# GreptimeTeam/greptimedb

Measured on AMD Instinct MI355X. Metric: TSBS DevOps ingest rows/sec (whole node), higher is better.
Workload: dtype f64; 1 GPU; model=tsbs-devops-cpu-only, global_batch=3000, seq_len=0, parallelism=region-shard dp1, scale_per_worker=100, workers=6, pool_rows=2394000, rows_shipped_cross_rank=0, wal=group-commit, no fsync, flush_mb=64, ssts_written=4, device=cuda:0

## Files before the change

### csrc/hip_ops.cpp

```cpp

#include <torch/extension.h>
#include <ATen/hip/HIPContext.h>

#include <algorithm>
#include <cmath>
#include <cstdint>
#include <tuple>
#include <vector>

#include "scatter_packed.h"

namespace gdb_hip {
void launch_ts_bucket_agg(
    const int64_t*, const int32_t*, const double*, int64_t, const int32_t*, int,
    const int32_t*, int, int64_t, int64_t, int64_t, int64_t, int, int, int64_t,
    double*, unsigned long long*, unsigned long long*, unsigned long long*,
    unsigned long long*, hipStream_t);
void launch_decode_minmax(
    const unsigned long long*, const unsigned long long*, const unsigned long long*,
    double*, double*, int64_t, hipStream_t);
void launch_filter_series_time(
    const int64_t*, const int32_t*, const int32_t*, int, int64_t, int64_t,
    int64_t, bool*, hipStream_t);
void launch_dedup_mark_last(const int32_t*, const int64_t*, int64_t, bool*, hipStream_t);
// ... 252 lines not shown
    CHECK_GPU(dst_ts[r]); CHECK_GPU(dst_se[r]); CHECK_GPU(dst_fields[r]);
    CHECK_CONTIG(dst_ts[r]); CHECK_CONTIG(dst_se[r]); CHECK_CONTIG(dst_fields[r]);
    TORCH_CHECK(dst_fields[r].dim() == 2 && dst_fields[r].size(0) >= nf,
                "region ", r, " has fewer field rows than the batch");
    TORCH_CHECK(bases[r] >= 0);
    regs.ts[r] = dst_ts[r].data_ptr<int64_t>();
    regs.se[r] = dst_se[r].data_ptr<int32_t>();
    regs.f[r] = dst_fields[r].data_ptr<double>();
    regs.stride[r] = dst_fields[r].size(1);
    regs.base[r] = bases[r];
    room[r] = std::min(std::min(dst_ts[r].numel(), dst_se[r].numel()),
                       dst_fields[r].size(1));
  }
  const uint8_t* hp = stage_pinned.data_ptr<uint8_t>();
  const int64_t* h_dst = reinterpret_cast<const int64_t*>(hp + off_dst);
  const int32_t* h_region = reinterpret_cast<const int32_t*>(hp + off_region);
  for (int64_t i = 0; i < n; i++) {
    const int32_t r = h_region[i];
    TORCH_CHECK(r >= 0 && r < R, "row ", i, ": region ", r, " out of range");
    TORCH_CHECK(h_dst[i] >= 0 && bases[r] + h_dst[i] < room[r],
                "row ", i, ": destination row beyond region ", r, " capacity");
  }
  auto stream = at::cuda::getCurrentHIPStream().stream();
  const hipError_t err = hipMemcpyAsync(
      stage_dev.data_ptr<uint8_t>(), hp, (size_t)used, hipMemcpyHostToDevice, stream);
  TORCH_CHECK(err == hipSuccess, "stage upload failed: ", hipGetErrorString(err));
  gdb_hip::launch_scatter_append_packed(
      stage_dev.data_ptr<uint8_t>(), n, (int)nf, regs, stream);
  const hipError_t lerr = hipGetLastError();
  TORCH_CHECK(lerr == hipSuccess, "scatter_append_packed launch failed: ",
              hipGetErrorString(lerr));
}

torch::Tensor rle_expand_indices(torch::Tensor runs, torch::Tensor blob,
                                 int64_t bw, int64_t n) {
  CHECK_GPU(runs); CHECK_CONTIG(runs); CHECK_GPU(blob); CHECK_CONTIG(blob);
  auto out = torch::empty({n}, blob.options().dtype(torch::kInt32));
  auto stream = at::cuda::getCurrentHIPStream().stream();
  gdb_hip::launch_rle_expand_indices(
      runs.data_ptr<int64_t>(), runs.size(0), blob.data_ptr<uint8_t>(),
      (int)bw, out.data_ptr<int32_t>(), n, stream);
  return out;
}

std::vector<torch::Tensor> gorilla_decode(torch::Tensor blob,
                                          torch::Tensor block_off,
                                          torch::Tensor out_off, int64_t n) {
  CHECK_GPU(blob); CHECK_CONTIG(blob);
  CHECK_GPU(block_off); CHECK_GPU(out_off);
  auto ts = torch::empty({n}, blob.options().dtype(torch::kInt64));
  auto vals = torch::empty({n}, blob.options().dtype(torch::kFloat64));
  auto stream = at::cuda::getCurrentHIPStream().stream();
// ... 181 lines not shown
```

### csrc/native.cpp

```cpp

#include <pybind11/pybind11.h>
#include <pybind11/numpy.h>
#include <pybind11/stl.h>

#include <cerrno>
#include <cmath>
#include <cstdint>
#include <cstring>
#include <fcntl.h>
#include <stdexcept>
#include <string>
#include <unistd.h>
#include <unordered_map>
#include <vector>

#include "ingest_core.h"

namespace py = pybind11;

static uint32_t crc_table[8][256];
static bool crc_init_done = [] {
  for (uint32_t i = 0; i < 256; i++) {
    uint32_t c = i;
    for (int k = 0; k < 8; k++) c = (c & 1) ? 0xEDB88320u ^ (c >> 1) : c >> 1;
    crc_table[0][i] = c;
  }
  for (int t = 1; t < 8; t++)
    for (uint32_t i = 0; i < 256; i++)
      crc_table[t][i] = crc_table[0][crc_table[t - 1][i] & 0xFF] ^
                        (crc_table[t - 1][i] >> 8);
  return true;
}();

static uint32_t crc32_update(uint32_t crc, const uint8_t* buf, size_t len) {
  crc = ~crc;
  while (len >= 8) {
    uint32_t lo, hi;
    std::memcpy(&lo, buf, 4);
    std::memcpy(&hi, buf + 4, 4);
    lo ^= crc;
    crc = crc_table[7][lo & 0xFF] ^ crc_table[6][(lo >> 8) & 0xFF] ^
          crc_table[5][(lo >> 16) & 0xFF] ^ crc_table[4][lo >> 24] ^
          crc_table[3][hi & 0xFF] ^ crc_table[2][(hi >> 8) & 0xFF] ^
          crc_table[1][(hi >> 16) & 0xFF] ^ crc_table[0][hi >> 24];
    buf += 8;
    len -= 8;
  }
  for (size_t i = 0; i < len; i++)
    crc = crc_table[0][(crc ^ buf[i]) & 0xFF] ^ (crc >> 8);
  return ~crc;
}

static inline uint64_t fnv1a(const char* p, size_t n) {
  uint64_t h = 1469598103934665603ULL;
  for (size_t i = 0; i < n; i++) { h ^= (uint8_t)p[i]; h *= 1099511628211ULL; }
  return h;
}


static py::capsule owner_of(void* p) {
  return py::capsule(p, [](void* q) { std::free(q); });
}

class LineParser {
 public:
  py::tuple parse(py::bytes data) {
    char* buf;
    Py_ssize_t len;
    if (PyBytes_AsStringAndSize(data.ptr(), &buf, &len) != 0)
      throw std::runtime_error("expected bytes");
    gdb_ingest::ParseSink sink;
    const size_t F0 = core_.num_fields();
    size_t nrows = 0, est = 0;
    int32_t* series = nullptr;
// ... 120 lines not shown
        py::array_t<double> a((py::ssize_t)n);
        if (n) {
          if (c < sink.col.size()) {
            std::memcpy(a.mutable_data(), sink.col[c], 8 * n);
          } else {
            std::fill(a.mutable_data(), a.mutable_data() + n, std::nan(""));
          }
        }
        fields[py::str(names[c])] = std::move(a);
      }
    }
    py::list newts;
    for (auto& [id, s] : sink.new_tagsets)
      newts.append(py::make_tuple(id, py::bytes(s)));
    return py::make_tuple(std::move(series), std::move(ts), std::move(fields),
                          std::move(newts));
  }

  gdb_ingest::LineCore core_;
};



class WalWriter {
 public:
  WalWriter() = default;
  ~WalWriter() { close_segment(); }

  void open_segment(const std::string& path) {
    close_segment();
    fd_ = ::open(path.c_str(), O_CREAT | O_WRONLY | O_APPEND, 0644);
    if (fd_ < 0) throw std::runtime_error("wal open failed: " + path + ": " + strerror(errno));
    path_ = path;
    seg_bytes_ = ::lseek(fd_, 0, SEEK_END);
  }

  void close_segment() {
    if (fd_ >= 0) { ::close(fd_); fd_ = -1; }
  }

  void append(uint64_t region_id, uint64_t seq, py::object payload) {
    char* pbuf; Py_ssize_t plen;
    Py_buffer view;
    bool have_view = false;
    if (PyBytes_Check(payload.ptr())) {
      if (PyBytes_AsStringAndSize(payload.ptr(), &pbuf, &plen) != 0)
        throw std::runtime_error("payload must be bytes");
    } else {
      if (PyObject_GetBuffer(payload.ptr(), &view, PyBUF_SIMPLE) != 0)
        throw py::error_already_set();
      have_view = true;
      pbuf = static_cast<char*>(view.buf);
      plen = view.len;
    }
    struct Release {
      Py_buffer* v;
      ~Release() { if (v) PyBuffer_Release(v); }
    } release{have_view ? &view : nullptr};
    py::gil_scoped_release rel;
    uint32_t body_len = 16 + static_cast<uint32_t>(plen);
    size_t off = buf_.size();
    buf_.resize(off + 8 + body_len);
    uint8_t* w = buf_.data() + off;
    std::memcpy(w, &body_len, 4);
    uint8_t hdr[16];
    std::memcpy(hdr, &region_id, 8);
    std::memcpy(hdr + 8, &seq, 8);
    uint32_t crc = crc32_update(0, hdr, 16);
    crc = crc32_update(crc, reinterpret_cast<uint8_t*>(pbuf), plen);
    std::memcpy(w + 4, &crc, 4);
    std::memcpy(w + 8, hdr, 16);
    std::memcpy(w + 24, pbuf, plen);
  }

  uint64_t commit(bool sync) {
    if (fd_ < 0) throw std::runtime_error("wal: no open segment");
    size_t n = buf_.size();
    if (n) {
      py::gil_scoped_release rel;
      const uint8_t* p = buf_.data();
      size_t left = n;
      while (left) {
        ssize_t w = ::write(fd_, p, left);
        if (w < 0) {
          if (errno == EINTR) continue;
          throw std::runtime_error(std::string("wal write failed: ") + strerror(errno));
        }
        p += w; left -= w;
      }
      if (sync && ::fdatasync(fd_) != 0)
        throw std::runtime_error(std::string("wal fdatasync failed: ") + strerror(errno));
    }
    buf_.clear();
    seg_bytes_ += n;
    return seg_bytes_;
  }

  uint64_t segment_bytes() const { return seg_bytes_; }

 private:
  int fd_ = -1;
  std::string path_;
  uint64_t seg_bytes_ = 0;
  std::vector<uint8_t> buf_;
};

static py::list wal_read_segment(const std::string& path) {
  py::list out;
  int fd = ::open(path.c_str(), O_RDONLY);
  if (fd < 0) throw std::runtime_error("wal open failed: " + path);
  off_t sz = ::lseek(fd, 0, SEEK_END);
  ::lseek(fd, 0, SEEK_SET);
  std::vector<uint8_t> data(sz);
  size_t got = 0;
  while (got < static_cast<size_t>(sz)) {
    ssize_t r = ::read(fd, data.data() + got, sz - got);
    if (r <= 0) break;
    got += r;
  }
  ::close(fd);
  size_t off = 0;
  while (off + 8 <= got) {
    uint32_t body_len, crc;
    std::memcpy(&body_len, data.data() + off, 4);
    std::memcpy(&crc, data.data() + off + 4, 4);
    if (body_len < 16 || off + 8 + body_len > got) break;
    const uint8_t* body = data.data() + off + 8;
    if (crc32_update(0, body, body_len) != crc) break;
    uint64_t region, seq;
    std::memcpy(&region, body, 8);
    std::memcpy(&seq, body + 8, 8);
    out.append(py::make_tuple(region, seq,
        py::bytes(reinterpret_cast<const char*>(body + 16), body_len - 16)));
    off += 8 + body_len;
  }
  return out;
}


static bool snappy_uncompress(const uint8_t* in, size_t n, std::vector<uint8_t>& out) {
  size_t ip = 0;
  uint64_t ulen = 0;
  int shift = 0;
  while (ip < n) {
    uint8_t b = in[ip++];
    ulen |= (uint64_t)(b & 0x7F) << shift;
    if (!(b & 0x80)) break;
    shift += 7;
    if (shift > 35) return false;
  }
  out.clear();
  out.reserve(ulen);
  while (ip < n) {
    const uint8_t tag = in[ip++];
    const int type = tag & 3;
    if (type == 0) {
      size_t len = (tag >> 2) + 1;
      if (len > 60) {
        const int extra = (int)len - 60;
// ... 945 lines not shown
                        std::move(counts), std::move(mins), std::move(maxs));
}

void register_pagedec(py::module_& m);

PYBIND11_MODULE(_native, m) {
  register_pagedec(m);
  m.doc() = "greptimedb_amd host-native ingest path (line parser + WAL)";
  py::class_<LineParser>(m, "LineParser")
      .def(py::init<>())
      .def("parse", &LineParser::parse)
      .def("ingest_batch", &LineParser::ingest_batch, py::arg("data"),
           py::arg("sid_region"), py::arg("sid_local"), py::arg("fmap"),
           py::arg("n_parser_fields"), py::arg("n_regions"),
           py::arg("hdr_suffix"), py::arg("durable"), py::arg("ts_scale"),
           py::arg("stage"))
      .def("num_fields", &LineParser::num_fields)
      .def("intern_capacity", &LineParser::intern_capacity)
      .def("num_series", &LineParser::num_series)
      .def("tagset_str", &LineParser::tagset_str)
      .def("field_names", &LineParser::field_names)
      .def("register_tagset", &LineParser::register_tagset)
      .def("register_field", &LineParser::register_field);
  py::class_<WalWriter>(m, "WalWriter")
      .def(py::init<>())
      .def("open_segment", &WalWriter::open_segment)
      .def("close_segment", &WalWriter::close_segment)
      .def("append", &WalWriter::append)
      .def("commit", &WalWriter::commit, py::arg("sync") = true)
      .def("segment_bytes", &WalWriter::segment_bytes);
  m.def("wal_read_segment", &wal_read_segment);
  m.def("snappy_uncompress", &py_snappy_uncompress);
  m.def("pack_str_col", &pack_str_col);
  m.def("route_ingest", &route_ingest, "K16 host-side ingest router");
  py::class_<PromWriteParser>(m, "PromWriteParser")
      .def(py::init<>())
      .def("parse", &PromWriteParser::parse, py::arg("data"), py::arg("is_snappy") = true)
      .def("num_series", &PromWriteParser::num_series);
  py::class_<OtlpMetricsParser>(m, "OtlpMetricsParser")
      .def(py::init<>())
      .def("parse", &OtlpMetricsParser::parse);
  py::class_<OtlpLogsParser>(m, "OtlpLogsParser")
      .def(py::init<>())
      .def("parse", &OtlpLogsParser::parse);
  py::class_<OtlpTraceParser>(m, "OtlpTraceParser")
      .def(py::init<>())
      .def("parse", &OtlpTraceParser::parse)
      .def("num_series", &OtlpTraceParser::num_series);
  py::class_<Tokenizer>(m, "Tokenizer")
      .def(py::init<>())
      .def("tokenize", &Tokenizer::tokenize)
      .def("term_id", &Tokenizer::term_id)
      .def("intern", &Tokenizer::intern)
// ... 5 lines not shown
```

### greptimedb_amd/engine/engine.py

```python

from __future__ import annotations

import json
import os
import queue
import threading
from dataclasses import dataclass, field

import numpy as np

from greptimedb_amd.engine.region import Region
from greptimedb_amd.engine.wal import Wal, decode_batch, encode_batch
from greptimedb_amd.models.schema import TableSchema, region_id as make_region_id
from greptimedb_amd.utils.errors import TableAlreadyExists, TableNotFound


@dataclass
class EngineConfig:
    data_dir: str = "./greptime_data"
    device: str = "cpu"
    flush_bytes: int = 512 << 20
    wal_sync: bool = False
    wal_segment_bytes: int = 256 << 20
    wal_shards: int = 1
    default_regions: int = 4
    background_flush: bool = True
    scan_mem_bytes: int = 32 << 30
    record_events: bool = False
    gc_interval_s: float = 600.0
    gc_grace_s: float = 3600.0
    cold_compress_s: float = 0.0
    global_write_buffer_bytes: int = 16 << 30


@dataclass
class TableState:
    schema: TableSchema
    regions: list = field(default_factory=list)
    append_mode: bool = False
    rule: object = None


class MitoEngine:
    def __init__(self, config: EngineConfig):
        self.config = config
        os.makedirs(config.data_dir, exist_ok=True)
        self.tables: dict[str, TableState] = {}
        self.next_table_id = 1024
        self._ddl_lock = threading.Lock()
        self._catalog_path = os.path.join(config.data_dir, "catalog.json")
        self.wal = Wal(os.path.join(config.data_dir, "wal"),
                       segment_bytes=config.wal_segment_bytes,
                       sync_on_commit=config.wal_sync,
                       shards=config.wal_shards)
        self._flush_q: queue.Queue = queue.Queue()
        self._flusher = None
        self.write_listeners: list = []
        self.flush_listeners: list = []
        self.mirror_listeners: list = []
        from greptimedb_amd.utils.memquota import MemoryQuota
        self.scan_quota = MemoryQuota(config.scan_mem_bytes)
        self._load_catalog()
        self._replay_wal()
# ... 274 lines not shown
                mem.max_ts = mx if mem.max_ts is None else max(mem.max_ts, mx)
                region.last_seq = max(region.last_seq, seqs[k])
                region.row_seq += m
        finally:
            for r in reversed(ordered):
                r.lock.release()
        if self.mirror_listeners and n:
            fnames = table.regions[0].field_names
            for k, region in enumerate(regions):
                if int(counts[k]) == 0:
                    continue
                rows = np.flatnonzero(region_of == k)
                for cb in self.mirror_listeners:
                    cb(table, region, series_codes[rows], ts_ms[rows],
                       fields[:, rows], fnames)
        if self.write_listeners and n:
            lo, hi = int(np.min(ts_ms)), int(np.max(ts_ms))
            for cb in self.write_listeners:
                cb(table.schema.name, lo, hi, n)
        return True

    def write_regions_fused(self, table: TableState, slot, n: int, nf: int,
                            counts, mins, maxs, payloads: list,
                            durable: bool = True) -> None:
        import torch
        from greptimedb_amd.ops import cpu_ref
        from greptimedb_amd.ops import kernels as ops

        regions: list[Region] = table.regions
        counts = [int(c) for c in counts]
        seqs = [0] * len(regions)
        if durable:
            for k, p in enumerate(payloads):
                if p is not None:
                    seqs[k] = self.wal.append(regions[k].region_id, p)
        ordered = sorted(regions, key=lambda r: r.region_id)
        for r in ordered:
            r.lock.acquire()
        try:
            bases = []
            for k, region in enumerate(regions):
                mem = region.memtable
                if mem.nf < nf:
                    mem.add_fields(nf - mem.nf)
                need = mem.len + counts[k]
                if need > mem.cap:
                    mem._grow(need)
                bases.append(mem.len)
            dst_ts = [r.memtable.ts for r in regions]
            dst_se = [r.memtable.series for r in regions]
            dst_f = [r.memtable.fields for r in regions]
            if slot.dev is not None:
                ops.scatter_append_packed(slot.host, slot.dev, n, nf, bases,
                                          dst_ts, dst_se, dst_f)
                if slot.event is not None:
                    slot.event.record()
            else:
                ts_h, f_h, do_h, se_h, ro_h = cpu_ref.packed_segments(
                    slot.host, n, nf)
                dev = self.config.device
                dst = do_h + torch.tensor(bases, dtype=torch.int64)[ro_h.long()]
                ops.scatter_append(ts_h.to(dev), se_h.to(dev), f_h.to(dev),
                                   ro_h.to(dev), dst.to(dev),
                                   dst_ts, dst_se, dst_f)
            for k, region in enumerate(regions):
                m = counts[k]
                if m == 0:
                    continue
                mem = region.memtable
                mem.len = bases[k] + m
                mn, mx = int(mins[k]), int(maxs[k])
                mem.min_ts = mn if mem.min_ts is None else min(mem.min_ts, mn)
                mem.max_ts = mx if mem.max_ts is None else max(mem.max_ts, mx)
                region.last_seq = max(region.last_seq, seqs[k])
                region.row_seq += m
        finally:
            for r in reversed(ordered):
                r.lock.release()
        if (self.mirror_listeners or self.write_listeners) and n:
            ts_h, f_h, _do, se_h, ro_h = (
                t.numpy() for t in cpu_ref.packed_segments(slot.host, n, nf))
            if self.mirror_listeners:
                fnames = table.regions[0].field_names
                for k, region in enumerate(regions):
                    if counts[k] == 0:
                        continue
                    rows = np.flatnonzero(ro_h == k)
                    for cb in self.mirror_listeners:
                        cb(table, region, se_h[rows], ts_h[rows],
                           f_h[:, rows], fnames)
            if self.write_listeners:
                lo, hi = int(np.min(ts_h)), int(np.max(ts_h))
                for cb in self.write_listeners:
                    cb(table.schema.name, lo, hi, n)
# ... 203 lines not shown
```

### greptimedb_amd/engine/ingest.py

```python

from __future__ import annotations

import weakref

import numpy as np

from greptimedb_amd import _native
from greptimedb_amd.engine.engine import MitoEngine, TableState
from greptimedb_amd.engine.series import tsid_hash
from greptimedb_amd.models.schema import ColumnSchema, DataType, SemanticType, TableSchema


def parse_tagset(key: bytes) -> tuple[str, list[tuple[str, str]]]:
    parts = key.decode().split(",")
    measurement = parts[0]
    tags = []
    for p in parts[1:]:
        if "=" in p:
            k, v = p.split("=", 1)
            tags.append((k, v))
    return measurement, tags


STAGE_RING = 3
# ... 18 lines not shown
                slot.event.synchronize()
            except Exception:
                pass
            slot.busy = False


class Ingestor:
    def __init__(self, engine: MitoEngine, default_regions: int | None = None,
                 append_mode: bool = True, durable: bool = True,
                 rank: int = 0, world: int = 1, exchange=None):
        self.engine = engine
        self.parser = _native.LineParser()
        self.append_mode = append_mode
        self.durable = durable
        self.default_regions = default_regions or engine.config.default_regions
        self.rank = rank
        self.world = world
        self.exchange = exchange
        self._remote_cache: dict[bytes, tuple[int, int]] = {}
        self._remote_lock = __import__("threading").Lock()
        self._bulk = engine.config.device.startswith("cuda")
        self._fused = True
        self._packed = True
        self._ring: list[_StageSlot] = []
        self._ring_pos = 0
        self._fused_st = None
        self._fused_lut = None
        weakref.finalize(self, _drain_ring, self._ring)
        self._cap = 1024
        self.sid_region = np.full(self._cap, -1, dtype=np.int32)
        self.sid_local = np.full(self._cap, -1, dtype=np.int32)
        self.sid_rank = np.full(self._cap, -1, dtype=np.int32)
        self.sid_key = np.empty(self._cap, dtype=object)
        self.flat_regions: list = []
        self._region_key: dict = {}
        self._table_field_map: dict = {}
        self._wal_suffix_cache: dict = {}
        self._flat_ridx_cache = None
        self._flat_ridx_table = None
        self.rows_ingested = 0
        self.rows_shipped = 0

    def _flat_region(self, st: TableState, region_idx: int) -> int:
        key = (st.schema.name, region_idx)
        idx = self._region_key.get(key)
        if idx is None:
# ... 172 lines not shown
        lut = self._fused_lut or self._build_fused_lut(st0)
        fmap = cached[0]
        nf = len(fmap)
        suffix = self._wal_suffix(st0)
        if not self._ring:
            self._grow_ring(1 << 16)
        res = None
        for _attempt in range(2):
            slot = self._next_slot()
            res = self.parser.ingest_batch(
                data, lut[0], lut[1], fmap, nparse, len(regions), suffix,
                self.durable, int(ts_scale_to_ns), slot.np)
            if res[0] != 2:
                break
            self._grow_ring(int(res[1]))
        if res[0] == 2:
            raise RuntimeError("ingest stage block still too small after growing")
        if res[0] == 1:
            return res[1]
        _, n, counts, mins, maxs, payloads = res
        if n == 0:
            return 0
        engine = self.engine
        engine.write_regions_fused(st0, slot, n, nf, counts, mins, maxs,
                                   payloads, durable=self.durable)
        slot.busy = slot.event is not None
        self._ring_pos = (self._ring_pos + 1) % len(self._ring)
        if self.durable:
            engine.commit_wal()
        engine.maybe_flush()
        self.rows_ingested += n
        return n

    def ingest_lines(self, data: bytes, ts_scale_to_ns: int = 1) -> int:
        if self._bulk and self._fused:
            got = self._ingest_fused(data, ts_scale_to_ns)
            if isinstance(got, int):
                return got
            series, ts_ns, fields, new_tagsets = got
        else:
            series, ts_ns, fields, new_tagsets = self.parser.parse(data)
        n = len(series)
        if n == 0:
            return 0
        self._check_epoch()
        for sid, key in new_tagsets:
            self._register_tagset(sid, key)
        rank_of = self.sid_rank[series]
        if bool((rank_of < 0).any()):
            for sid in np.unique(series[rank_of < 0]):
                self._register_tagset(int(sid), self.parser.tagset_str(int(sid)))
# ... 212 lines not shown
```

### greptimedb_amd/engine/wal.py

```python

from __future__ import annotations

import heapq
import json
import os
import re
import struct
import threading

import numpy as np

from greptimedb_amd import _native


def encode_batch(series: np.ndarray, ts_ms: np.ndarray, fields: np.ndarray,
                 field_names: list[str], new_series: list[tuple[int, bytes]],
                 str_cols: dict[str, list] | None = None) -> bytes:
    str_cols = str_cols or {}
    bin_cols = [name for name, vals in str_cols.items()
                if any(isinstance(v, (bytes, bytearray)) for v in vals)]
    hdr = json.dumps({
        "n": int(len(ts_ms)),
        "fields": field_names,
        "strs": list(str_cols),
# ... 93 lines not shown
    def _shard_of(self, region_id: int) -> _Shard:
        return self.shards[region_id % len(self.shards)]

    def append(self, region_id: int, payload: bytes) -> int:
        with self._lock:
            seq = self.next_seq
            self.next_seq += 1
            self.region_last[region_id] = seq
        sh = self._shard_of(region_id)
        with sh.lock:
            sh.writer.append(region_id, seq, payload)
            sh.dirty = True
        return seq

    def commit(self):
        for sh in self.shards:
            if not sh.dirty:
                continue
            with sh.lock:
                if not sh.dirty:
                    continue
                size = sh.writer.commit(self.sync_on_commit)
                sh.dirty = False
                if size >= self.segment_bytes:
                    sh.writer.close_segment()
                    sh.writer.open_segment(sh.seg_path(self.next_seq))

    def replay(self):
        def shard_stream(shard_idx):
            for seg in self.segments(shard_idx):
                for region, seq, payload in _native.wal_read_segment(
                        os.path.join(self.dir, seg)):
                    yield seq, seg, region, payload

        streams = [shard_stream(i) for i in range(len(self.shards))]
        present = {int(_SEG_RE.match(f).group(2) or 0) for f in self.segments()}
        for extra in sorted(present - set(range(len(self.shards)))):
            streams.append(shard_stream(extra))
        for seq, seg, region, payload in heapq.merge(*streams):
            yield seg, region, seq, payload

    def purge_before(self, seq: int):
        for sh in range(len(self.shards)):
            segs = self.segments(sh)
            for i, seg in enumerate(segs[:-1]):
                nxt_first = int(_SEG_RE.match(segs[i + 1]).group(1))
                if nxt_first <= seq:
                    os.unlink(os.path.join(self.dir, seg))

    def close(self):
        for sh in self.shards:
            if sh.writer is None:
                continue
            try:
                sh.writer.commit(self.sync_on_commit)
            except RuntimeError:
                pass
            sh.writer.close_segment()
            sh.writer = None
        self.shards = []
```

Measured before the change: 14.70 million rows/s.

## Batch WAL append+commit natively, add CLMUL CRC, release GIL around upload

Moves the WAL writer into a shared C++ header and adds a native append-and-commit call that frames and writes all region payloads of a fused batch in one GIL-free pass, replacing the per-region Python append loop plus a separate commit. Adds a PCLMUL-based CRC32 path for payloads of 64 bytes or more, caches the sorted region order and converts count/min/max arrays with tolist. It also releases the GIL around the H2D stage copy and scatter launch. The WAL path now writes immediately per batch instead of buffering, and rotation and sync semantics change.

Result: faster. 16.64 million rows/s (median of 6 runs) (+13.2%).

```diff
diff --git a/csrc/hip_ops.cpp b/csrc/hip_ops.cpp
--- a/csrc/hip_ops.cpp
+++ b/csrc/hip_ops.cpp
@@ -298,12 +298,17 @@
                 "row ", i, ": destination row beyond region ", r, " capacity");
   }
   auto stream = at::cuda::getCurrentHIPStream().stream();
-  const hipError_t err = hipMemcpyAsync(
-      stage_dev.data_ptr<uint8_t>(), hp, (size_t)used, hipMemcpyHostToDevice, stream);
+  uint8_t* dp = stage_dev.data_ptr<uint8_t>();
+  hipError_t err = hipSuccess, lerr = hipSuccess;
+  {
+    py::gil_scoped_release nogil;
+    err = hipMemcpyAsync(dp, hp, (size_t)used, hipMemcpyHostToDevice, stream);
+    if (err == hipSuccess) {
+      gdb_hip::launch_scatter_append_packed(dp, n, (int)nf, regs, stream);
+      lerr = hipGetLastError();
+    }
+  }
   TORCH_CHECK(err == hipSuccess, "stage upload failed: ", hipGetErrorString(err));
-  gdb_hip::launch_scatter_append_packed(
-      stage_dev.data_ptr<uint8_t>(), n, (int)nf, regs, stream);
-  const hipError_t lerr = hipGetLastError();
   TORCH_CHECK(lerr == hipSuccess, "scatter_append_packed launch failed: ",
               hipGetErrorString(lerr));
 }
diff --git a/csrc/native.cpp b/csrc/native.cpp
--- a/csrc/native.cpp
+++ b/csrc/native.cpp
@@ -15,41 +15,11 @@
 #include <vector>
 
 #include "ingest_core.h"
+#include "wal_core.h"
 
 namespace py = pybind11;
 
-static uint32_t crc_table[8][256];
-static bool crc_init_done = [] {
-  for (uint32_t i = 0; i < 256; i++) {
-    uint32_t c = i;
-    for (int k = 0; k < 8; k++) c = (c & 1) ? 0xEDB88320u ^ (c >> 1) : c >> 1;
-    crc_table[0][i] = c;
-  }
-  for (int t = 1; t < 8; t++)
-    for (uint32_t i = 0; i < 256; i++)
-      crc_table[t][i] = crc_table[0][crc_table[t - 1][i] & 0xFF] ^
-                        (crc_table[t - 1][i] >> 8);
-  return true;
-}();
-
-static uint32_t crc32_update(uint32_t crc, const uint8_t* buf, size_t len) {
-  crc = ~crc;
-  while (len >= 8) {
-    uint32_t lo, hi;
-    std::memcpy(&lo, buf, 4);
-    std::memcpy(&hi, buf + 4, 4);
-    lo ^= crc;
-    crc = crc_table[7][lo & 0xFF] ^ crc_table[6][(lo >> 8) & 0xFF] ^
-          crc_table[5][(lo >> 16) & 0xFF] ^ crc_table[4][lo >> 24] ^
-          crc_table[3][hi & 0xFF] ^ crc_table[2][(hi >> 8) & 0xFF] ^
-          crc_table[1][(hi >> 16) & 0xFF] ^ crc_table[0][hi >> 24];
-    buf += 8;
-    len -= 8;
-  }
-  for (size_t i = 0; i < len; i++)
-    crc = crc_table[0][(crc ^ buf[i]) & 0xFF] ^ (crc >> 8);
-  return ~crc;
-}
+using gdb_wal::crc32_update;
 
 static inline uint64_t fnv1a(const char* p, size_t n) {
   uint64_t h = 1469598103934665603ULL;
@@ -216,119 +186,112 @@
 
 
 
-class WalWriter {
- public:
-  WalWriter() = default;
-  ~WalWriter() { close_segment(); }
-
-  void open_segment(const std::string& path) {
-    close_segment();
-    fd_ = ::open(path.c_str(), O_CREAT | O_WRONLY | O_APPEND, 0644);
-    if (fd_ < 0) throw std::runtime_error("wal open failed: " + path + ": " + strerror(errno));
-    path_ = path;
-    seg_bytes_ = ::lseek(fd_, 0, SEEK_END);
-  }
-
-  void close_segment() {
-    if (fd_ >= 0) { ::close(fd_); fd_ = -1; }
-  }
-
-  void append(uint64_t region_id, uint64_t seq, py::object payload) {
-    char* pbuf; Py_ssize_t plen;
-    Py_buffer view;
-    bool have_view = false;
-    if (PyBytes_Check(payload.ptr())) {
-      if (PyBytes_AsStringAndSize(payload.ptr(), &pbuf, &plen) != 0)
+struct PayloadView {
+  const uint8_t* p = nullptr;
+  size_t n = 0;
+  Py_buffer view;
+  bool have_view = false;
+  py::object owner;
+
+  PayloadView() = default;
+  PayloadView(const PayloadView&) = delete;
+  PayloadView& operator=(const PayloadView&) = delete;
+  ~PayloadView() { if (have_view) PyBuffer_Release(&view); }
+
+  void acquire(PyObject* o) {
+    owner = py::reinterpret_borrow<py::object>(o);
+    if (PyBytes_Check(o)) {
+      char* b; Py_ssize_t len;
+      if (PyBytes_AsStringAndSize(o, &b, &len) != 0)
         throw std::runtime_error("payload must be bytes");
+      p = reinterpret_cast<const uint8_t*>(b);
+      n = (size_t)len;
     } else {
-      if (PyObject_GetBuffer(payload.ptr(), &view, PyBUF_SIMPLE) != 0)
+      if (PyObject_GetBuffer(o, &view, PyBUF_SIMPLE) != 0)
         throw py::error_already_set();
       have_view = true;
-      pbuf = static_cast<char*>(view.buf);
-      plen = view.len;
-    }
-    struct Release {
-      Py_buffer* v;
-      ~Release() { if (v) PyBuffer_Release(v); }
-    } release{have_view ? &view : nullptr};
+      p = static_cast<const uint8_t*>(view.buf);
+      n = (size_t)view.len;
+    }
+  }
+};
+
+static void wal_writer_append(gdb_wal::WalWriter& w, uint64_t region_id,
+                              uint64_t seq, py::object payload) {
+  PayloadView v;
+  v.acquire(payload.ptr());
+  py::gil_scoped_release rel;
+  w.append(region_id, seq, v.p, v.n);
+}
+
+static py::list wal_append_commit(py::list writers,
+                                  std::vector<uint64_t> region_ids,
+                                  std::vector<uint64_t> seqs,
+                                  py::list payloads, bool sync) {
+  const size_t m = (size_t)py::len(writers);
+  if (region_ids.size() != m || seqs.size() != m || (size_t)py::len(payloads) != m)
+    throw std::runtime_error("wal_append_commit: argument lists differ in length");
+  std::vector<gdb_wal::WalWriter*> w(m);
+  std::vector<py::object> writer_refs(m);
+  std::vector<PayloadView> views(m);
+  for (size_t i = 0; i < m; i++) {
+    writer_refs[i] = writers[i];
+    w[i] = py::cast<gdb_wal::WalWriter*>(writer_refs[i]);
+    if (w[i] == nullptr)
+      throw std::runtime_error("wal_append_commit: writer is None");
+    views[i].acquire(py::object(payloads[i]).ptr());
+  }
+  std::vector<uint64_t> sizes(m, 0);
+  std::string error;
+  {
     py::gil_scoped_release rel;
-    uint32_t body_len = 16 + static_cast<uint32_t>(plen);
-    size_t off = buf_.size();
-    buf_.resize(off + 8 + body_len);
-    uint8_t* w = buf_.data() + off;
-    std::memcpy(w, &body_len, 4);
-    uint8_t hdr[16];
-    std::memcpy(hdr, &region_id, 8);
-    std::memcpy(hdr + 8, &seq, 8);
-    uint32_t crc = crc32_update(0, hdr, 16);
-    crc = crc32_update(crc, reinterpret_cast<uint8_t*>(pbuf), plen);
-    std::memcpy(w + 4, &crc, 4);
-    std::memcpy(w + 8, hdr, 16);
-    std::memcpy(w + 24, pbuf, plen);
-  }
-
-  uint64_t commit(bool sync) {
-    if (fd_ < 0) throw std::runtime_error("wal: no open segment");
-    size_t n = buf_.size();
-    if (n) {
-      py::gil_scoped_release rel;
-      const uint8_t* p = buf_.data();
-      size_t left = n;
-      while (left) {
-        ssize_t w = ::write(fd_, p, left);
-        if (w < 0) {
-          if (errno == EINTR) continue;
-          throw std::runtime_error(std::string("wal write failed: ") + strerror(errno));
-        }
-        p += w; left -= w;
-      }
-      if (sync && ::fdatasync(fd_) != 0)
-        throw std::runtime_error(std::string("wal fdatasync failed: ") + strerror(errno));
-    }
-    buf_.clear();
-    seg_bytes_ += n;
-    return seg_bytes_;
-  }
-
-  uint64_t segment_bytes() const { return seg_bytes_; }
-
- private:
-  int fd_ = -1;
-  std::string path_;
-  uint64_t seg_bytes_ = 0;
-  std::vector<uint8_t> buf_;
-};
+    try {
+      std::vector<uint8_t> hdrs(m * gdb_wal::kFrameHeaderBytes);
+      for (size_t i = 0; i < m; i++)
+        gdb_wal::frame_header(hdrs.data() + i * gdb_wal::kFrameHeaderBytes,
+                              region_ids[i], seqs[i], views[i].p, views[i].n);
+      for (size_t i = 0; i < m; i++) {
+        bool last_of_writer = true;
+        for (size_t j = i + 1; j < m && last_of_writer; j++)
+          last_of_writer = w[j] != w[i];
+        sizes[i] = w[i]->append_commit(
+            hdrs.data() + i * gdb_wal::kFrameHeaderBytes, views[i].p,
+            views[i].n, sync && last_of_writer);
+      }
+    } catch (const std::exception& e) {
+      error = e.what();
+      if (error.empty()) error = "wal_append_commit failed";
+    }
+  }
+  if (!error.empty()) throw std::runtime_error(error);
+  py::list out;
+  for (size_t i = 0; i < m; i++) out.append(py::int_(sizes[i]));
+  return out;
+}
 
 static py::list wal_read_segment(const std::string& path) {
+  std::vector<uint8_t> data;
+  std::vector<gdb_wal::FrameView> frames;
+  {
+    py::gil_scoped_release rel;
+    data = gdb_wal::read_file(path);
+    frames = gdb_wal::read_frames(data.data(), data.size());
+  }
   py::list out;
-  int fd = ::open(path.c_str(), O_RDONLY);
-  if (fd < 0) throw std::runtime_error("wal open failed: " + path);
-  off_t sz = ::lseek(fd, 0, SEEK_END);
-  ::lseek(fd, 0, SEEK_SET);
-  std::vector<uint8_t> data(sz);
-  size_t got = 0;
-  while (got < static_cast<size_t>(sz)) {
-    ssize_t r = ::read(fd, data.data() + got, sz - got);
-    if (r <= 0) break;
-    got += r;
-  }
-  ::close(fd);
-  size_t off = 0;
-  while (off + 8 <= got) {
-    uint32_t body_len, crc;
-    std::memcpy(&body_len, data.data() + off, 4);
-    std::memcpy(&crc, data.data() + off + 4, 4);
-    if (body_len < 16 || off + 8 + body_len > got) break;
-    const uint8_t* body = data.data() + off + 8;
-    if (crc32_update(0, body, body_len) != crc) break;
-    uint64_t region, seq;
-    std::memcpy(&region, body, 8);
-    std::memcpy(&seq, body + 8, 8);
-    out.append(py::make_tuple(region, seq,
-        py::bytes(reinterpret_cast<const char*>(body + 16), body_len - 16)));
-    off += 8 + body_len;
-  }
+  for (const auto& f : frames)
+    out.append(py::make_tuple(
+        f.region, f.seq,
+        py::bytes(reinterpret_cast<const char*>(f.payload), f.plen)));
   return out;
+}
+
+static uint32_t py_crc32(py::object data, uint32_t init, const std::string& impl) {
+  PayloadView v;
+  v.acquire(data.ptr());
+  if (impl == "auto") return gdb_wal::crc32_update(init, v.p, v.n);
+  if (impl == "table") return gdb_wal::crc32_table(init, v.p, v.n);
+  if (impl == "clmul") return gdb_wal::crc32_clmul(init, v.p, v.n);
+  throw std::invalid_argument("crc32: impl must be auto, table or clmul");
 }
 
 
@@ -1320,13 +1283,32 @@
       .def("field_names", &LineParser::field_names)
       .def("register_tagset", &LineParser::register_tagset)
       .def("register_field", &LineParser::register_field);
-  py::class_<WalWriter>(m, "WalWriter")
+  py::class_<gdb_wal::WalWriter>(m, "WalWriter")
       .def(py::init<>())
-      .def("open_segment", &WalWriter::open_segment)
-      .def("close_segment", &WalWriter::close_segment)
-      .def("append", &WalWriter::append)
-      .def("commit", &WalWriter::commit, py::arg("sync") = true)
-      .def("segment_bytes", &WalWriter::segment_bytes);
+      .def("open_segment", &gdb_wal::WalWriter::open_segment,
+           py::call_guard<py::gil_scoped_release>())
+      .def("close_segment", &gdb_wal::WalWriter::close_segment,
+           py::arg("sync") = false, py::call_guard<py::gil_scoped_release>())
+      .def("rotate", &gdb_wal::WalWriter::rotate, py::arg("path"),
+           py::arg("sync") = false, py::call_guard<py::gil_scoped_release>())
+      .def("append", &wal_writer_append)
+      .def("commit", &gdb_wal::WalWriter::commit, py::arg("sync") = true,
+           py::call_guard<py::gil_scoped_release>())
+      .def("segment_bytes", &gdb_wal::WalWriter::segment_bytes,
+           py::call_guard<py::gil_scoped_release>())
+      .def("unsynced_bytes", &gdb_wal::WalWriter::unsynced_bytes,
+           py::call_guard<py::gil_scoped_release>())
+      .def("sync_count", &gdb_wal::WalWriter::sync_count,
+           py::call_guard<py::gil_scoped_release>());
+  m.def("wal_append_commit", &wal_append_commit, py::arg("writers"),
+        py::arg("region_ids"), py::arg("seqs"), py::arg("payloads"),
+        py::arg("sync") = false);
+  m.def("crc32", &py_crc32, py::arg("data"), py::arg("init") = 0,
+        py::arg("impl") = "auto");
+  m.def("crc32_have_clmul", &gdb_wal::crc32_have_clmul);
+  m.def("crc32_force_table", [](bool on) {
+    gdb_wal::crc32_force_table_flag().store(on);
+  }, "measurement switch: make the \"auto\" CRC path use the table");
   m.def("wal_read_segment", &wal_read_segment);
   m.def("snappy_uncompress", &py_snappy_uncompress);
   m.def("pack_str_col", &pack_str_col);
diff --git a/csrc/wal_core.h b/csrc/wal_core.h
--- /dev/null
+++ b/csrc/wal_core.h
@@ -0,0 +1,379 @@
+#pragma once
+
+#include <atomic>
+#include <cerrno>
+#include <cstdint>
+#include <cstring>
+#include <fcntl.h>
+#include <mutex>
+#include <stdexcept>
+#include <string>
+#include <sys/uio.h>
+#include <unistd.h>
+#include <vector>
+
+#if defined(__x86_64__) && (defined(__GNUC__) || defined(__clang__))
+#define GDB_WAL_HAVE_CLMUL_BUILD 1
+#include <immintrin.h>
+#else
+#define GDB_WAL_HAVE_CLMUL_BUILD 0
+#endif
+
+namespace gdb_wal {
+
+
+struct CrcTables {
+  uint32_t t[8][256];
+  CrcTables() {
+    for (uint32_t i = 0; i < 256; i++) {
+      uint32_t c = i;
+      for (int k = 0; k < 8; k++) c = (c & 1) ? 0xEDB88320u ^ (c >> 1) : c >> 1;
+      t[0][i] = c;
+    }
+    for (int s = 1; s < 8; s++)
+      for (uint32_t i = 0; i < 256; i++)
+        t[s][i] = t[0][t[s - 1][i] & 0xFF] ^ (t[s - 1][i] >> 8);
+  }
+};
+
+inline const CrcTables& crc_tables() {
+  static const CrcTables tables;
+  return tables;
+}
+
+inline uint32_t crc32_table_raw(uint32_t crc, const uint8_t* buf, size_t len) {
+  const auto& T = crc_tables().t;
+  while (len >= 8) {
+    uint32_t lo, hi;
+    std::memcpy(&lo, buf, 4);
+    std::memcpy(&hi, buf + 4, 4);
+    lo ^= crc;
+    crc = T[7][lo & 0xFF] ^ T[6][(lo >> 8) & 0xFF] ^
+          T[5][(lo >> 16) & 0xFF] ^ T[4][lo >> 24] ^
+          T[3][hi & 0xFF] ^ T[2][(hi >> 8) & 0xFF] ^
+          T[1][(hi >> 16) & 0xFF] ^ T[0][hi >> 24];
+    buf += 8;
+    len -= 8;
+  }
+  for (size_t i = 0; i < len; i++)
+    crc = T[0][(crc ^ buf[i]) & 0xFF] ^ (crc >> 8);
+  return crc;
+}
+
+inline uint32_t crc32_table(uint32_t crc, const uint8_t* buf, size_t len) {
+  return ~crc32_table_raw(~crc, buf, len);
+}
+
+inline bool crc32_have_clmul() {
+#if GDB_WAL_HAVE_CLMUL_BUILD
+  static const bool have = __builtin_cpu_supports("pclmul") &&
+                           __builtin_cpu_supports("sse4.1");
+  return have;
+#else
+  return false;
+#endif
+}
+
+#if GDB_WAL_HAVE_CLMUL_BUILD
+#define GDB_WAL_CLMUL_FN __attribute__((target("pclmul,sse4.1"))) inline
+
+GDB_WAL_CLMUL_FN __m128i clmul_load(const uint8_t* p) {
+  return _mm_loadu_si128(reinterpret_cast<const __m128i*>(p));
+}
+
+GDB_WAL_CLMUL_FN __m128i clmul_fold(__m128i lane, __m128i k, __m128i next) {
+  const __m128i lo = _mm_clmulepi64_si128(lane, k, 0x00);
+  const __m128i hi = _mm_clmulepi64_si128(lane, k, 0x11);
+  return _mm_xor_si128(_mm_xor_si128(lo, hi), next);
+}
+
+GDB_WAL_CLMUL_FN uint32_t crc32_clmul_raw(uint32_t crc, const uint8_t* buf,
+                                          size_t len) {
+  const __m128i k1k2 = _mm_set_epi64x(0x01c6e41596, 0x0154442bd4);
+  const __m128i k3k4 = _mm_set_epi64x(0x00ccaa009e, 0x01751997d0);
+  const __m128i k5 = _mm_set_epi64x(0, 0x0163cd6124);
+  const __m128i poly_mu = _mm_set_epi64x(0x01f7011641, 0x01db710641);
+  const __m128i low32 = _mm_set_epi32(0, ~0, 0, ~0);
+  __m128i a = _mm_xor_si128(clmul_load(buf), _mm_cvtsi32_si128((int)crc));
+  __m128i b = clmul_load(buf + 16), c = clmul_load(buf + 32), d = clmul_load(buf + 48);
+  buf += 64;
+  len -= 64;
+  while (len >= 64) {
+    a = clmul_fold(a, k1k2, clmul_load(buf));
+    b = clmul_fold(b, k1k2, clmul_load(buf + 16));
+    c = clmul_fold(c, k1k2, clmul_load(buf + 32));
+    d = clmul_fold(d, k1k2, clmul_load(buf + 48));
+    buf += 64;
+    len -= 64;
+  }
+  a = clmul_fold(a, k3k4, b);
+  a = clmul_fold(a, k3k4, c);
+  a = clmul_fold(a, k3k4, d);
+  while (len >= 16) {
+    a = clmul_fold(a, k3k4, clmul_load(buf));
+    buf += 16;
+    len -= 16;
+  }
+  __m128i t = _mm_clmulepi64_si128(a, k3k4, 0x10);
+  a = _mm_xor_si128(_mm_srli_si128(a, 8), t);
+  t = _mm_srli_si128(a, 4);
+  a = _mm_clmulepi64_si128(_mm_and_si128(a, low32), k5, 0x00);
+  a = _mm_xor_si128(a, t);
+  t = _mm_clmulepi64_si128(_mm_and_si128(a, low32), poly_mu, 0x10);
+  t = _mm_clmulepi64_si128(_mm_and_si128(t, low32), poly_mu, 0x00);
+  a = _mm_xor_si128(a, t);
+  return (uint32_t)_mm_extract_epi32(a, 1);
+}
+#endif
+
+inline uint32_t crc32_clmul(uint32_t crc, const uint8_t* buf, size_t len) {
+#if GDB_WAL_HAVE_CLMUL_BUILD
+  if (!crc32_have_clmul())
+    throw std::runtime_error("crc32: this CPU has no pclmul + sse4.1");
+  crc = ~crc;
+  if (len >= 64) {
+    const size_t head = len & ~(size_t)15;
+    crc = crc32_clmul_raw(crc, buf, head);
+    buf += head;
+    len -= head;
+  }
+  return ~crc32_table_raw(crc, buf, len);
+#else
+  (void)crc; (void)buf; (void)len;
+  throw std::runtime_error("crc32: built without pclmul support");
+#endif
+}
+
+inline std::atomic<bool>& crc32_force_table_flag() {
+  static std::atomic<bool> force{false};
+  return force;
+}
+
+inline uint32_t crc32_update(uint32_t crc, const uint8_t* buf, size_t len) {
+  if (len >= 64 && crc32_have_clmul() &&
+      !crc32_force_table_flag().load(std::memory_order_relaxed))
+    return crc32_clmul(crc, buf, len);
+  return crc32_table(crc, buf, len);
+}
+
+
+constexpr size_t kFrameHeaderBytes = 24;
+
+inline void frame_header(uint8_t out[kFrameHeaderBytes], uint64_t region_id,
+                         uint64_t seq, const uint8_t* payload, size_t plen) {
+  if (plen > 0xFFFFFFFFull - 16)
+    throw std::runtime_error("wal: payload too large for one frame");
+  const uint32_t body_len = 16 + static_cast<uint32_t>(plen);
+  std::memcpy(out, &body_len, 4);
+  std::memcpy(out + 8, &region_id, 8);
+  std::memcpy(out + 16, &seq, 8);
+  uint32_t crc = crc32_update(0, out + 8, 16);
+  crc = crc32_update(crc, payload, plen);
+  std::memcpy(out + 4, &crc, 4);
+}
+
+
+class WalWriter {
+ public:
+  WalWriter() = default;
+  WalWriter(const WalWriter&) = delete;
+  WalWriter& operator=(const WalWriter&) = delete;
+  ~WalWriter() {
+    try { close_segment(); } catch (...) {}
+  }
+
+  void open_segment(const std::string& path) {
+    std::lock_guard<std::mutex> g(mu_);
+    open_locked(path);
+  }
+
+  void close_segment(bool sync = false) {
+    std::lock_guard<std::mutex> g(mu_);
+    close_locked(sync);
+  }
+
+  void rotate(const std::string& path, bool sync = false) {
+    std::lock_guard<std::mutex> g(mu_);
+    open_locked(path, sync);
+  }
+
+  void append(uint64_t region_id, uint64_t seq, const uint8_t* payload,
+              size_t plen) {
+    uint8_t hdr[kFrameHeaderBytes];
+    frame_header(hdr, region_id, seq, payload, plen);
+    std::lock_guard<std::mutex> g(mu_);
+    const size_t off = buf_.size();
+    buf_.resize(off + kFrameHeaderBytes + plen);
+    std::memcpy(buf_.data() + off, hdr, kFrameHeaderBytes);
+    if (plen) std::memcpy(buf_.data() + off + kFrameHeaderBytes, payload, plen);
+  }
+
+  uint64_t commit(bool sync) {
+    std::lock_guard<std::mutex> g(mu_);
+    if (fd_ < 0) throw std::runtime_error("wal: no open segment");
+    flush_locked();
+    if (sync) sync_locked();
+    return seg_bytes_;
+  }
+
+  uint64_t append_commit(const uint8_t hdr[kFrameHeaderBytes],
+                         const uint8_t* payload, size_t plen, bool sync) {
+    std::lock_guard<std::mutex> g(mu_);
+    if (fd_ < 0) throw std::runtime_error("wal: no open segment");
+    flush_locked();
+    size_t done = 0;
+    const size_t total = kFrameHeaderBytes + plen;
+    while (done < total) {
+      struct iovec iov[2];
+      int cnt = 0;
+      if (done < kFrameHeaderBytes) {
+        iov[cnt].iov_base = const_cast<uint8_t*>(hdr) + done;
+        iov[cnt].iov_len = kFrameHeaderBytes - done;
+        cnt++;
+        if (plen) {
+          iov[cnt].iov_base = const_cast<uint8_t*>(payload);
+          iov[cnt].iov_len = plen;
+          cnt++;
+        }
+      } else {
+        const size_t poff = done - kFrameHeaderBytes;
+        iov[cnt].iov_base = const_cast<uint8_t*>(payload) + poff;
+        iov[cnt].iov_len = plen - poff;
+        cnt++;
+      }
+      const ssize_t w = ::writev(fd_, iov, cnt);
+      if (w < 0) {
+        if (errno == EINTR) continue;
+        seg_bytes_ += done;
+        unsynced_ += done;
+        throw std::runtime_error(std::string("wal write failed: ") +
+                                 strerror(errno));
+      }
+      done += static_cast<size_t>(w);
+    }
+    seg_bytes_ += total;
+    unsynced_ += total;
+    if (sync) sync_locked();
+    return seg_bytes_;
+  }
+
+  uint64_t segment_bytes() {
+    std::lock_guard<std::mutex> g(mu_);
+    return seg_bytes_;
+  }
+
+  uint64_t unsynced_bytes() {
+    std::lock_guard<std::mutex> g(mu_);
+    return unsynced_;
+  }
+
+  uint64_t sync_count() {
+    std::lock_guard<std::mutex> g(mu_);
+    return sync_count_;
+  }
+
+ private:
+  void close_locked(bool sync) {
+    if (fd_ < 0) return;
+    if (sync) sync_locked();
+    else if (want_sync_ && unsynced_) sync_locked();
+    ::close(fd_);
+    fd_ = -1;
+    unsynced_ = 0;
+  }
+
+  void open_locked(const std::string& path, bool sync = false) {
+    const int fd = ::open(path.c_str(), O_CREAT | O_WRONLY | O_APPEND, 0644);
+    if (fd < 0)
+      throw std::runtime_error("wal open failed: " + path + ": " + strerror(errno));
+    try {
+      close_locked(sync);
+    } catch (...) {
+      ::close(fd);
+      throw;
+    }
+    fd_ = fd;
+    seg_bytes_ = static_cast<uint64_t>(::lseek(fd_, 0, SEEK_END));
+  }
+
+  void flush_locked() {
+    const uint8_t* p = buf_.data();
+    size_t left = buf_.size();
+    while (left) {
+      const ssize_t w = ::write(fd_, p, left);
+      if (w < 0) {
+        if (errno == EINTR) continue;
+        throw std::runtime_error(std::string("wal write failed: ") + strerror(errno));
+      }
+      p += w;
+      left -= static_cast<size_t>(w);
+    }
+    seg_bytes_ += buf_.size();
+    unsynced_ += buf_.size();
+    buf_.clear();
+  }
+
+  void sync_locked() {
+    want_sync_ = true;
+    if (unsynced_ == 0) return;
+    if (::fdatasync(fd_) != 0)
+      throw std::runtime_error(std::string("wal fdatasync failed: ") + strerror(errno));
+    sync_count_++;
+    unsynced_ = 0;
+  }
+
+  std::mutex mu_;
+  int fd_ = -1;
+  uint64_t seg_bytes_ = 0;
+  uint64_t unsynced_ = 0;
+  uint64_t sync_count_ = 0;
+  bool want_sync_ = false;
+  std::vector<uint8_t> buf_;
+};
+
+struct FrameView {
+  uint64_t region, seq;
+  const uint8_t* payload;
+  size_t plen;
+};
+
+inline std::vector<FrameView> read_frames(const uint8_t* data, size_t n) {
+  std::vector<FrameView> out;
+  size_t off = 0;
+  while (off + 8 <= n) {
+    uint32_t body_len, crc;
+    std::memcpy(&body_len, data + off, 4);
+    std::memcpy(&crc, data + off + 4, 4);
+    if (body_len < 16 || off + 8 + (size_t)body_len > n) break;
+    const uint8_t* body = data + off + 8;
+    if (crc32_update(0, body, body_len) != crc) break;
+    FrameView f;
+    std::memcpy(&f.region, body, 8);
+    std::memcpy(&f.seq, body + 8, 8);
+    f.payload = body + 16;
+    f.plen = body_len - 16;
+    out.push_back(f);
+    off += 8 + (size_t)body_len;
+  }
+  return out;
+}
+
+inline std::vector<uint8_t> read_file(const std::string& path) {
+  const int fd = ::open(path.c_str(), O_RDONLY);
+  if (fd < 0) throw std::runtime_error("wal open failed: " + path);
+  const off_t sz = ::lseek(fd, 0, SEEK_END);
+  ::lseek(fd, 0, SEEK_SET);
+  std::vector<uint8_t> data(sz > 0 ? (size_t)sz : 0);
+  size_t got = 0;
+  while (got < data.size()) {
+    const ssize_t r = ::read(fd, data.data() + got, data.size() - got);
+    if (r < 0 && errno == EINTR) continue;
+    if (r <= 0) break;
+    got += (size_t)r;
+  }
+  ::close(fd);
+  data.resize(got);
+  return data;
+}
+
+}
diff --git a/csrc/wal_core_check.cpp b/csrc/wal_core_check.cpp
--- /dev/null
+++ b/csrc/wal_core_check.cpp
@@ -0,0 +1,307 @@
+
+#include <atomic>
+#include <cstdio>
+#include <cstdlib>
+#include <map>
+#include <mutex>
+#include <string>
+#include <thread>
+#include <vector>
+
+#include "wal_core.h"
+
+using namespace gdb_wal;
+
+static std::atomic<int> failures{0};
+#define CHECK(cond)                                                    \
+  do {                                                                 \
+    if (!(cond)) {                                                     \
+      std::printf("CHECK failed %s:%d: %s\n", __FILE__, __LINE__, #cond); \
+      failures++;                                                      \
+    }                                                                  \
+  } while (0)
+
+
+static uint32_t crc32_bitwise(uint32_t crc, const uint8_t* p, size_t n) {
+  crc = ~crc;
+  for (size_t i = 0; i < n; i++) {
+    crc ^= p[i];
+    for (int k = 0; k < 8; k++) crc = (crc & 1) ? 0xEDB88320u ^ (crc >> 1) : crc >> 1;
+  }
+  return ~crc;
+}
+
+static void check_crc_one(const uint8_t* p, size_t n, uint32_t init) {
+  const uint32_t want = crc32_bitwise(init, p, n);
+  CHECK(crc32_table(init, p, n) == want);
+  CHECK(crc32_update(init, p, n) == want);
+  if (crc32_have_clmul()) CHECK(crc32_clmul(init, p, n) == want);
+}
+
+static void check_crc() {
+  const size_t big = 300001;
+  for (int fill = 0; fill < 3; fill++) {
+    std::vector<uint8_t> buf(big + 16);
+    uint32_t x = 0x9E3779B9u;
+    for (auto& b : buf) {
+      x = x * 1664525u + 1013904223u;
+      b = fill == 0 ? (uint8_t)(x >> 24) : fill == 1 ? 0x00 : 0xFF;
+    }
+    for (size_t n = 0; n <= 300; n++) {
+      std::vector<uint8_t> exact(buf.begin(), buf.begin() + n);
+      check_crc_one(exact.data(), n, 0);
+    }
+    for (size_t n : {(size_t)4095, (size_t)4096, (size_t)4097, big}) {
+      std::vector<uint8_t> exact(buf.begin(), buf.begin() + n);
+      check_crc_one(exact.data(), n, 0);
+      check_crc_one(exact.data(), n, 0xDEADBEEFu);
+    }
+    for (size_t off = 0; off < 16; off++) {
+      std::vector<uint8_t> exact(buf.begin(), buf.begin() + off + 1000);
+      check_crc_one(exact.data() + off, 1000, 0);
+      check_crc_one(exact.data() + off, 77, 12345u);
+    }
+  }
+  std::vector<uint8_t> buf(5000, 0xA5);
+  CHECK(crc32_update(crc32_update(0, buf.data(), 1234), buf.data() + 1234, 3766) ==
+        crc32_bitwise(0, buf.data(), 5000));
+}
+
+
+constexpr int kWriters = 2;
+constexpr int kThreads = 4;
+constexpr int kFramesPerThread = 400;
+constexpr uint64_t kSegmentBytes = 24 * 1024;
+
+static size_t payload_len(uint64_t seq) { return (size_t)((seq * 131) % 700); }
+static uint8_t payload_byte(uint64_t seq, size_t i) {
+  return (uint8_t)(seq * 7 + i * 13 + (i >> 8));
+}
+
+struct Shard {
+  WalWriter writer;
+  std::vector<std::string> segments;
+};
+
+static std::mutex seq_mu;
+static uint64_t next_seq = 1;
+static std::string dir;
+
+static std::string seg_path(int shard, uint64_t first_seq) {
+  char name[64];
+  std::snprintf(name, sizeof name, "/%020llu.s%d.wal",
+                (unsigned long long)first_seq, shard);
+  return dir + name;
+}
+
+static void maybe_rotate(Shard& sh, int idx, uint64_t size) {
+  if (size < kSegmentBytes) return;
+  std::lock_guard<std::mutex> g(seq_mu);
+  if (sh.writer.segment_bytes() < kSegmentBytes) return;
+  const std::string p = seg_path(idx, next_seq);
+  sh.writer.rotate(p);
+  sh.segments.push_back(p);
+}
+
+static void worker(Shard* shards, int tid) {
+  std::vector<uint8_t> payload;
+  for (int k = 0; k < kFramesPerThread; k++) {
+    uint64_t seq;
+    {
+      std::lock_guard<std::mutex> g(seq_mu);
+      seq = next_seq++;
+    }
+    const int idx = (int)((seq + (uint64_t)tid) % kWriters);
+    Shard& sh = shards[idx];
+    const uint64_t region = 4096 + (uint64_t)idx;
+    payload.resize(payload_len(seq));
+    for (size_t i = 0; i < payload.size(); i++) payload[i] = payload_byte(seq, i);
+    uint64_t size;
+    if (k % 3 == 0) {
+      sh.writer.append(region, seq, payload.data(), payload.size());
+      size = (k % 2 == 0) ? sh.writer.commit(false) : sh.writer.segment_bytes();
+    } else {
+      uint8_t hdr[kFrameHeaderBytes];
+      frame_header(hdr, region, seq, payload.data(), payload.size());
+      size = sh.writer.append_commit(hdr, payload.data(), payload.size(),
+                                     k % 50 == 1);
+    }
+    maybe_rotate(sh, idx, size);
+  }
+}
+
+static void check_writers() {
+  Shard shards[kWriters];
+  for (int i = 0; i < kWriters; i++) {
+    const std::string p = seg_path(i, 1);
+    shards[i].writer.open_segment(p);
+    shards[i].segments.push_back(p);
+  }
+  std::vector<std::thread> threads;
+  for (int t = 0; t < kThreads; t++) threads.emplace_back(worker, shards, t);
+  for (auto& t : threads) t.join();
+  for (auto& sh : shards) {
+    sh.writer.commit(true);
+    sh.writer.close_segment();
+  }
+
+  std::map<uint64_t, int> seen;
+  for (int i = 0; i < kWriters; i++) {
+    CHECK(shards[i].segments.size() >= 3);
+    uint64_t prev_first = 0;
+    for (size_t s = 0; s < shards[i].segments.size(); s++) {
+      const std::string& path = shards[i].segments[s];
+      const uint64_t first =
+          std::strtoull(path.substr(path.rfind('/') + 1, 20).c_str(), nullptr, 10);
+      CHECK(s == 0 || first >= prev_first);
+      const std::vector<uint8_t> data = read_file(path);
+      const std::vector<FrameView> frames = read_frames(data.data(), data.size());
+      size_t bytes = 0;
+      for (const auto& f : frames) {
+        bytes += kFrameHeaderBytes + f.plen;
+        seen[f.seq]++;
+        CHECK(f.region == 4096 + (uint64_t)i);
+        CHECK(f.plen == payload_len(f.seq));
+        if (s + 1 < shards[i].segments.size()) {
+          const std::string& nxt = shards[i].segments[s + 1];
+          CHECK(f.seq < std::strtoull(
+              nxt.substr(nxt.rfind('/') + 1, 20).c_str(), nullptr, 10));
+        }
+        bool same = f.plen == payload_len(f.seq);
+        for (size_t b = 0; same && b < f.plen; b++)
+          same = f.payload[b] == payload_byte(f.seq, b);
+        CHECK(same);
+      }
+      CHECK(bytes == data.size());
+      prev_first = first;
+    }
+  }
+  const uint64_t total = (uint64_t)kThreads * kFramesPerThread;
+  CHECK(seen.size() == total);
+  for (uint64_t s = 1; s <= total; s++) CHECK(seen.count(s) && seen[s] == 1);
+
+  WalWriter closed;
+  uint8_t hdr[kFrameHeaderBytes];
+  frame_header(hdr, 1, 1, nullptr, 0);
+  bool threw = false;
+  try { closed.append_commit(hdr, nullptr, 0, false); } catch (const std::runtime_error&) { threw = true; }
+  CHECK(threw);
+  threw = false;
+  try { closed.commit(false); } catch (const std::runtime_error&) { threw = true; }
+  CHECK(threw);
+  threw = false;
+  try { closed.rotate(dir + "/no/such/dir/x.wal"); } catch (const std::runtime_error&) { threw = true; }
+  CHECK(threw);
+}
+
+
+static void put(WalWriter& w, uint64_t seq, bool sync) {
+  const uint8_t payload[5] = {1, 2, 3, 4, 5};
+  uint8_t hdr[kFrameHeaderBytes];
+  frame_header(hdr, 7, seq, payload, sizeof payload);
+  w.append_commit(hdr, payload, sizeof payload, sync);
+}
+
+static void check_sync_order() {
+  const size_t frame = kFrameHeaderBytes + 5;
+  {
+    WalWriter w;
+    w.open_segment(dir + "/sync_a.wal");
+    put(w, 1, false);
+    put(w, 2, false);
+    put(w, 3, false);
+    CHECK(w.unsynced_bytes() == 3 * frame && w.sync_count() == 0);
+    w.rotate(dir + "/sync_b.wal", true);
+    CHECK(w.unsynced_bytes() == 0);
+    CHECK(w.sync_count() == 1);
+    put(w, 4, true);
+    CHECK(w.unsynced_bytes() == 0 && w.sync_count() == 2);
+    put(w, 5, false);
+    w.rotate(dir + "/sync_c.wal");
+    CHECK(w.unsynced_bytes() == 0 && w.sync_count() == 3);
+    put(w, 6, false);
+    w.close_segment();
+    CHECK(w.sync_count() == 4);
+    CHECK(read_frames(read_file(dir + "/sync_a.wal").data(), 3 * frame).size() == 3);
+  }
+  {
+    WalWriter w;
+    w.open_segment(dir + "/sync_d.wal");
+    const uint8_t payload[3] = {9, 9, 9};
+    w.append(7, 1, payload, sizeof payload);
+    put(w, 2, false);
+    CHECK(w.unsynced_bytes() == kFrameHeaderBytes + 3 + frame);
+    w.commit(true);
+    CHECK(w.unsynced_bytes() == 0 && w.sync_count() == 1);
+    w.commit(true);
+    CHECK(w.sync_count() == 1);
+    put(w, 3, true);
+    CHECK(w.sync_count() == 2);
+  }
+  {
+    WalWriter w;
+    w.open_segment(dir + "/sync_e.wal");
+    put(w, 1, false);
+    w.commit(false);
+    w.rotate(dir + "/sync_f.wal");
+    w.close_segment();
+    CHECK(w.sync_count() == 0);
+  }
+}
+
+static void check_sync_threads() {
+  WalWriter w;
+  std::mutex rot_mu;
+  int seg = 0;
+  std::atomic<uint64_t> seq{1};
+  w.open_segment(dir + "/sync_t0.wal");
+  auto body = [&](int tid) {
+    for (int k = 0; k < 40; k++) {
+      put(w, seq++, false);
+      put(w, seq++, false);
+      put(w, seq++, true);
+      if ((k + tid) % 5 == 0) {
+        std::lock_guard<std::mutex> g(rot_mu);
+        char name[48];
+        std::snprintf(name, sizeof name, "/sync_t%d.wal", ++seg);
+        w.rotate(dir + name, true);
+      }
+    }
+  };
+  std::vector<std::thread> threads;
+  for (int t = 0; t < kThreads; t++) threads.emplace_back(body, t);
+  for (auto& t : threads) t.join();
+  w.close_segment(true);
+  CHECK(w.unsynced_bytes() == 0);
+  size_t frames = 0;
+  for (int i = 0; i <= seg; i++) {
+    char name[48];
+    std::snprintf(name, sizeof name, "/sync_t%d.wal", i);
+    const std::vector<uint8_t> data = read_file(dir + name);
+    const size_t n = read_frames(data.data(), data.size()).size();
+    CHECK(n * (kFrameHeaderBytes + 5) == data.size());
+    frames += n;
+  }
+  CHECK(frames == (size_t)kThreads * 40 * 3);
+}
+
+int main(int argc, char** argv) {
+  if (argc > 1) {
+    dir = argv[1];
+  } else {
+    char tmpl[] = "/tmp/wal_core_check_XXXXXX";
+    const char* d = mkdtemp(tmpl);
+    if (!d) { std::perror("mkdtemp"); return 2; }
+    dir = d;
+  }
+  check_crc();
+  check_writers();
+  check_sync_order();
+  check_sync_threads();
+  if (failures.load()) {
+    std::printf("wal_core_check FAILED: %d\n", failures.load());
+    return 1;
+  }
+  std::printf("wal_core_check ok\n");
+  return 0;
+}
diff --git a/greptimedb_amd/engine/engine.py b/greptimedb_amd/engine/engine.py
--- a/greptimedb_amd/engine/engine.py
+++ b/greptimedb_amd/engine/engine.py
@@ -39,6 +39,7 @@
     regions: list = field(default_factory=list)
     append_mode: bool = False
     rule: object = None
+    fused_order: tuple = field(default=None, repr=False, compare=False)
 
 
 class MitoEngine:
@@ -359,19 +360,35 @@
 
     def write_regions_fused(self, table: TableState, slot, n: int, nf: int,
                             counts, mins, maxs, payloads: list,
-                            durable: bool = True) -> None:
+                            durable: bool = True,
+                            wal_batch: bool = False) -> None:
         import torch
         from greptimedb_amd.ops import cpu_ref
         from greptimedb_amd.ops import kernels as ops
 
         regions: list[Region] = table.regions
-        counts = [int(c) for c in counts]
+        cached = table.fused_order
+        if cached is None or cached[0] != regions:
+            cached = table.fused_order = (
+                list(regions),
+                tuple(sorted(regions, key=lambda r: r.region_id)),
+                tuple(r.region_id for r in regions))
+        ordered = cached[1]
+        counts, mins, maxs = (
+            a.tolist() if hasattr(a, "tolist") else [int(v) for v in a]
+            for a in (counts, mins, maxs))
         seqs = [0] * len(regions)
-        if durable:
+        if durable and wal_batch:
+            live = [k for k, p in enumerate(payloads) if p is not None]
+            rids = cached[2]
+            got = self.wal.append_commit_many(
+                [rids[k] for k in live], [payloads[k] for k in live])
+            for k, seq in zip(live, got):
+                seqs[k] = seq
+        elif durable:
             for k, p in enumerate(payloads):
                 if p is not None:
                     seqs[k] = self.wal.append(regions[k].region_id, p)
-        ordered = sorted(regions, key=lambda r: r.region_id)
         for r in ordered:
             r.lock.acquire()
         try:
@@ -406,7 +423,7 @@
                     continue
                 mem = region.memtable
                 mem.len = bases[k] + m
-                mn, mx = int(mins[k]), int(maxs[k])
+                mn, mx = mins[k], maxs[k]
                 mem.min_ts = mn if mem.min_ts is None else min(mem.min_ts, mn)
                 mem.max_ts = mx if mem.max_ts is None else max(mem.max_ts, mx)
                 region.last_seq = max(region.last_seq, seqs[k])
diff --git a/greptimedb_amd/engine/ingest.py b/greptimedb_amd/engine/ingest.py
--- a/greptimedb_amd/engine/ingest.py
+++ b/greptimedb_amd/engine/ingest.py
@@ -64,6 +64,7 @@
         self._bulk = engine.config.device.startswith("cuda")
         self._fused = True
         self._packed = True
+        self._wal_batch = True
         self._ring: list[_StageSlot] = []
         self._ring_pos = 0
         self._fused_st = None
@@ -282,11 +283,13 @@
         if n == 0:
             return 0
         engine = self.engine
+        wal_batch = self._wal_batch
         engine.write_regions_fused(st0, slot, n, nf, counts, mins, maxs,
-                                   payloads, durable=self.durable)
+                                   payloads, durable=self.durable,
+                                   wal_batch=wal_batch)
         slot.busy = slot.event is not None
         self._ring_pos = (self._ring_pos + 1) % len(self._ring)
-        if self.durable:
+        if self.durable and not wal_batch:
             engine.commit_wal()
         engine.maybe_flush()
         self.rows_ingested += n
diff --git a/greptimedb_amd/engine/wal.py b/greptimedb_amd/engine/wal.py
--- a/greptimedb_amd/engine/wal.py
+++ b/greptimedb_amd/engine/wal.py
@@ -139,9 +139,35 @@
                     continue
                 size = sh.writer.commit(self.sync_on_commit)
                 sh.dirty = False
-                if size >= self.segment_bytes:
-                    sh.writer.close_segment()
-                    sh.writer.open_segment(sh.seg_path(self.next_seq))
+            if size >= self.segment_bytes:
+                self._rotate(sh)
+
+    def _rotate(self, sh: _Shard):
+        with self._lock:
+            if sh.writer.segment_bytes() >= self.segment_bytes:
+                sh.writer.rotate(sh.seg_path(self.next_seq),
+                                 self.sync_on_commit)
+
+    def append_commit_many(self, region_ids: list[int],
+                           payloads: list) -> list[int]:
+        k = len(region_ids)
+        if k == 0:
+            return []
+        nsh = len(self.shards)
+        shards = [self.shards[r % nsh] for r in region_ids]
+        with self._lock:
+            first = self.next_seq
+            self.next_seq = first + k
+            seqs = list(range(first, first + k))
+            self.region_last.update(zip(region_ids, seqs))
+        sizes = _native.wal_append_commit(
+            [sh.writer for sh in shards], region_ids, seqs, payloads,
+            self.sync_on_commit)
+        limit = self.segment_bytes
+        for sh, size in zip(shards, sizes):
+            if size >= limit:
+                self._rotate(sh)
+        return seqs
 
     def replay(self):
         def shard_stream(shard_idx):
@@ -173,6 +199,6 @@
                 sh.writer.commit(self.sync_on_commit)
             except RuntimeError:
                 pass
-            sh.writer.close_segment()
+            sh.writer.close_segment(self.sync_on_commit)
             sh.writer = None
         self.shards = []
```
